# unionai-oss/unionml

Hardware: AMD Instinct MI355X
Metric: train_samples_per_sec (higher is better)
Workload: dtype bf16; 1 GPU; model=digits_mlp_64x32x10, global_batch=2048, parallelism=dp1, engine=fused+hipgraph64

## Files before the change

### unionml_amd/ops/hip/tabular_common.h

```cpp
#pragma once

#include <hip/hip_runtime.h>
#include <hip/hip_bf16.h>

#include "tabular_launch.h"

typedef __attribute__((ext_vector_type(8))) short bf16x8;
typedef __attribute__((ext_vector_type(4))) float f32x4;
typedef unsigned short u16;

constexpr int HEAD_XENT = 0;
constexpr int HEAD_REG = 1;

template <int HEAD> struct head_target { typedef int type; };
template <> struct head_target<HEAD_REG> { typedef float type; };
template <int HEAD> using head_target_t = typename head_target<HEAD>::type;

__device__ __forceinline__ float bf2f(u16 v) {
  union { float f; unsigned u; } c;
  c.u = ((unsigned)v) << 16;
  return c.f;
}

__device__ __forceinline__ u16 f2bf(float f) {
  union { float f; unsigned u; } c;
  c.f = f;
  unsigned lsb = (c.u >> 16) & 1u;
  c.u += 0x7fffu + lsb;
  return (u16)(c.u >> 16);
}

__device__ __forceinline__ float fast_rcp(float x) {
  return __builtin_amdgcn_rcpf(x);
}

template <int CTRL>
__device__ __forceinline__ float dpp_row_f32(float x) {
  return __int_as_float(__builtin_amdgcn_update_dpp(
      0, __float_as_int(x), CTRL, 0xF, 0xF, true));
}

__device__ __forceinline__ float row_sum16(float x) {
  x += dpp_row_f32<0xB1>(x);
  x += dpp_row_f32<0x4E>(x);
  x += dpp_row_f32<0x141>(x);
  x += dpp_row_f32<0x140>(x);
  return x;
}

template <int D>
__device__ __forceinline__ void group_pair(float x, float& a, float& b) {
  static_assert(D == 16 || D == 32, "row-of-16 or half-wave exchange");
  const int xi = __float_as_int(x);
  if constexpr (D == 16) {
    const auto r = __builtin_amdgcn_permlane16_swap(xi, xi, false, false);
    a = __int_as_float(r[0]);
    b = __int_as_float(r[1]);
  } else {
    const auto r = __builtin_amdgcn_permlane32_swap(xi, xi, false, false);
    a = __int_as_float(r[0]);
    b = __int_as_float(r[1]);
  }
}

template <int D>
__device__ __forceinline__ float group_sum(float x) {
  float a, b;
  group_pair<D>(x, a, b);
  return a + b;
}

template <int D>
__device__ __forceinline__ float group_max(float x) {
  float a, b;
  group_pair<D>(x, a, b);
  return fmaxf(a, b);
}


constexpr int tr_read_elem(int lane, int ks, int tile, int half, int stride) {
  const int lg = lane >> 4, lr = lane & 15;
  return (ks * 32 + lg * 8 + half * 4 + (lr >> 2)) * stride + tile * 16 + (lr & 3) * 4;
}

constexpr bool tr_read_map_ok(int stride, int KS, int TILES) {
  if (stride < TILES * 16) return false;
  for (int ks = 0; ks < KS; ++ks)
    for (int tile = 0; tile < TILES; ++tile)
      for (int half = 0; half < 2; ++half)
        for (int lane = 0; lane < 64; ++lane) {
          if ((tr_read_elem(lane, ks, tile, half, stride) * 2) % 8 != 0) return false;
          const int group = lane & ~15, i = lane & 15;
          for (int q = 0; q < 4; ++q) {
            const int got = tr_read_elem(group + 4 * q + (i >> 2), ks, tile, half, stride) + (i & 3);
            const int want_row = ks * 32 + (lane >> 4) * 8 + half * 4 + q;
            const int want_col = tile * 16 + i;
            if (got / stride != want_row || got % stride != want_col) return false;
          }
        }
  return true;
}

template <int STRIDE, int KS, int TILES>
__device__ __forceinline__ bf16x8 tr_read_k8(const u16 (*T)[STRIDE], int ks, int tile,
                                             int lane) {
  static_assert(tr_read_map_ok(STRIDE, KS, TILES), "transposed-read address map");
  typedef __attribute__((ext_vector_type(4))) short s16x4;
  typedef __attribute__((address_space(3))) s16x4 lds_s16x4;
  const u16* base = &T[0][0];
  const s16x4 lo = __builtin_amdgcn_ds_read_tr16_b64_v4i16(
      (lds_s16x4*)(base + tr_read_elem(lane, ks, tile, 0, STRIDE)));
  const s16x4 hi = __builtin_amdgcn_ds_read_tr16_b64_v4i16(
      (lds_s16x4*)(base + tr_read_elem(lane, ks, tile, 1, STRIDE)));
  return __builtin_shufflevector(lo, hi, 0, 1, 2, 3, 4, 5, 6, 7);
}


typedef __attribute__((address_space(1))) float xwg_f32;
typedef __attribute__((address_space(1))) unsigned xwg_u32;

__device__ __forceinline__ void xwg_store(float* p, float x) {
  __hip_atomic_store((xwg_f32*)p, x, __ATOMIC_RELAXED, __HIP_MEMORY_SCOPE_AGENT);
}
__device__ __forceinline__ void xwg_store(unsigned* p, unsigned x) {
  __hip_atomic_store((xwg_u32*)p, x, __ATOMIC_RELAXED, __HIP_MEMORY_SCOPE_AGENT);
}
__device__ __forceinline__ float xwg_load(const float* p) {
  return __hip_atomic_load((const xwg_f32*)p, __ATOMIC_RELAXED, __HIP_MEMORY_SCOPE_AGENT);
}
__device__ __forceinline__ unsigned xwg_load(const unsigned* p) {
  return __hip_atomic_load((const xwg_u32*)p, __ATOMIC_RELAXED, __HIP_MEMORY_SCOPE_AGENT);
}

__device__ __forceinline__ void xwg_store4(float* base, int n, int i, f32x4 x) {
  typedef __attribute__((ext_vector_type(4))) unsigned u32x4;
  const __amdgpu_buffer_rsrc_t rsrc =
      __builtin_amdgcn_make_buffer_rsrc(base, 0, n * 4, 0x00020000);
  __builtin_amdgcn_raw_buffer_store_b128(__builtin_bit_cast(u32x4, x), rsrc, i * 4, 0, 16);
}


__device__ __forceinline__ float adam_corr(float beta_pow_t) {
  return fast_rcp(1.f - beta_pow_t);
}

__device__ __forceinline__ void adam_bias_corr(float beta1, float beta2, float t,
                                               float& corr1, float& corr2) {
  corr1 = adam_corr(__powf(beta1, t));
  corr2 = adam_corr(__powf(beta2, t));
}

__device__ __forceinline__ void adam_update(float& p, float& m, float& v, float g,
                                            float lr, float beta1, float beta2,
                                            float eps, float corr1, float corr2) {
  const float omb1 = 1.f - beta1, omb2 = 1.f - beta2;
  float bm, bv, gs;
  {
    #pragma clang fp contract(off)
    bm = beta1 * m;
    bv = beta2 * v;
    gs = omb2 * g;
  }
  const float mi = __builtin_fmaf(omb1, g, bm);
  const float vi = __builtin_fmaf(g, gs, bv);
  m = mi;
  v = vi;
  p = p - lr * (mi * corr1) * fast_rcp(sqrtf(vi * corr2) + eps);
}


__device__ __forceinline__ void wimg_write(u16* __restrict__ wimg, int i, u16 wb) {
  static_assert(DIGITS_HID == 32 && DIGITS_CPAD == 16, "shifts below");
  if (i < DIGITS_OFF_B1) {
    const int in = i >> 5;
    const int h = i & 31;
    wimg[DIGITS_WIMG_W1T + h * DIGITS_XS + in] = wb;
  } else if (i >= DIGITS_OFF_W2 && i < DIGITS_OFF_B2) {
    const int j = i - DIGITS_OFF_W2;
    const int h = j >> 4;
    const int c = j & 15;
    wimg[DIGITS_WIMG_W2S + h * DIGITS_WS + c] = wb;
    wimg[DIGITS_WIMG_W2T + c * DIGITS_WS + h] = wb;
  }
}

__device__ __forceinline__ int wimg_w2s_off(int hid, int inp) { return hid * inp; }
__device__ __forceinline__ int wimg_w2t_off(int hid, int inp) {
  return hid * inp + hid * 32;
}

__device__ __forceinline__ void wimg_write_gen(u16* __restrict__ wimg, int inp,
                                               int hid, int cpad, int i, u16 wb) {
  const int off_b1 = inp * hid;
  const int off_w2 = off_b1 + hid;
  const int off_b2 = off_w2 + hid * cpad;
  if (i < off_b1) {
    wimg[(i % hid) * inp + (i / hid)] = wb;
  } else if (i >= off_w2 && i < off_b2) {
    const int j = i - off_w2;
    const int h = j / cpad, c = j % cpad;
    wimg[wimg_w2s_off(hid, inp) + h * 32 + c] = wb;
    wimg[wimg_w2t_off(hid, inp) + c * hid + h] = wb;
  }
}


template <int NCT>
__device__ __forceinline__ void head_logits(float (&logit)[NCT][4],
                                            const f32x4 (&acc)[NCT],
                                            const float* b2, int cls, int lg) {
  #pragma unroll
  for (int ct = 0; ct < NCT; ++ct) {
    #pragma unroll
    for (int r = 0; r < 4; ++r) {
      const int c = ct * 16 + lg * 4 + r;
      logit[ct][r] = (c < cls) ? acc[ct][r] + b2[c] : -1e30f;
    }
  }
}

__device__ __forceinline__ void head_logits_padded(float (&logit)[1][4],
                                                   const f32x4 (&acc)[1],
                                                   f32x4 b2v, int cls, int lg) {
  #pragma unroll
  for (int r = 0; r < 4; ++r) {
    const int c = lg * 4 + r;
    logit[0][r] = (c < cls) ? acc[0][r] + b2v[r] : -1e30f;
  }
}

template <int NCT>
__device__ __forceinline__ float head_row_max(const float (&logit)[NCT][4]) {
  float mx = -1e30f;
  #pragma unroll
  for (int ct = 0; ct < NCT; ++ct) {
    #pragma unroll
    for (int r = 0; r < 4; ++r) mx = fmaxf(mx, logit[ct][r]);
  }
  mx = group_max<16>(mx);
  mx = group_max<32>(mx);
  return mx;
}

template <int NCT>
__device__ __forceinline__ float head_exp_sum(float (&e)[NCT][4],
                                              const float (&logit)[NCT][4],
                                              float mx, int cls, int lg) {
  float s = 0.f;
  #pragma unroll
  for (int ct = 0; ct < NCT; ++ct) {
    #pragma unroll
    for (int r = 0; r < 4; ++r) {
      const int c = ct * 16 + lg * 4 + r;
      e[ct][r] = (c < cls) ? __expf(logit[ct][r] - mx) : 0.f;
      s += e[ct][r];
    }
  }
  s = group_sum<16>(s);
  s = group_sum<32>(s);
  return s;
}

template <int NCT>
__device__ __forceinline__ void head_argmax(const float (&logit)[NCT][4], int cls,
                                            int lg, float& best, int& bcol) {
  best = -1e30f;
  bcol = cls;
  #pragma unroll
  for (int ct = 0; ct < NCT; ++ct) {
    #pragma unroll
    for (int r = 0; r < 4; ++r) {
      if (logit[ct][r] > best) { best = logit[ct][r]; bcol = ct * 16 + lg * 4 + r; }
    }
  }
  #pragma unroll
  for (int d = 16; d < 64; d <<= 1) {
    const float ov = __shfl_xor(best, d, 64);
    const int oc = __shfl_xor(bcol, d, 64);
    if (ov > best || (ov == best && oc < bcol)) { best = ov; bcol = oc; }
  }
}
```

### unionml_amd/ops/hip/tabular_kernels.hip

```cpp

#include <hip/hip_runtime.h>

#include "tabular_common.h"

constexpr int IN = DIGITS_IN, HID = DIGITS_HID, CLS = DIGITS_CLS;
constexpr int CPAD = DIGITS_CPAD;
#define ROWS 128
#define WAVES 8
#define BLOCK (WAVES * 64)

constexpr int XS = DIGITS_XS;
#define HS 40
#define DHS 36
constexpr int WS = DIGITS_WS;


extern "C" __global__ void __launch_bounds__(256)
standardize_fit_fast_kernel(const float* __restrict__ X, long long N, int D,
                            double* __restrict__ scratch ) {
  const int tid = threadIdx.x;
  const int col = tid % D;
  const int rg = tid / D;
  const int rpi = 256 / D;
  double s = 0.0, s2 = 0.0;
  for (long long r = (long long)blockIdx.x * rpi + rg; r < N;
       r += (long long)gridDim.x * rpi) {
    const double v = (double)X[r * D + col];
    s += v;
    s2 += v * v;
  }
  __shared__ double ls[256], ls2[256];
  ls[tid] = s;
  ls2[tid] = s2;
  __syncthreads();
  for (int off = 128; off >= D; off >>= 1) {
    if (tid < off && tid + off < 256) {
      ls[tid] += ls[tid + off];
      ls2[tid] += ls2[tid + off];
    }
    __syncthreads();
  }
  if (tid < D) {
    atomicAdd(&scratch[col], ls[tid]);
    atomicAdd(&scratch[D + col], ls2[tid]);
  }
}

extern "C" __global__ void __launch_bounds__(256)
standardize_fit_finalize_kernel(const double* __restrict__ scratch, long long N,
                                int D, float* __restrict__ mean,
                                float* __restrict__ invstd, float eps) {
  const int col = blockIdx.x * blockDim.x + threadIdx.x;
  if (col >= D) return;
  const double m = scratch[col] / (double)N;
  const double var = scratch[D + col] / (double)N - m * m;
  mean[col] = (float)m;
  invstd[col] = (float)(1.0 / sqrt(var > 0.0 ? var + (double)eps : (double)eps));
}

extern "C" __global__ void __launch_bounds__(256)
standardize_fit_kernel(const float* __restrict__ X, long long N, int D,
                       float* __restrict__ mean, float* __restrict__ invstd,
                       float eps) {
  const int col = blockIdx.x;
  if (col >= D) return;
  double s = 0.0, s2 = 0.0;
  for (long long r = threadIdx.x; r < N; r += blockDim.x) {
    const double v = (double)X[r * D + col];
    s += v;
    s2 += v * v;
  }
  __shared__ double ls[256], ls2[256];
  ls[threadIdx.x] = s;
  ls2[threadIdx.x] = s2;
  __syncthreads();
  for (int off = 128; off > 0; off >>= 1) {
    if (threadIdx.x < off) {
      ls[threadIdx.x] += ls[threadIdx.x + off];
      ls2[threadIdx.x] += ls2[threadIdx.x + off];
    }
    __syncthreads();
  }
  if (threadIdx.x == 0) {
    const double m = ls[0] / (double)N;
    const double var = ls2[0] / (double)N - m * m;
    mean[col] = (float)m;
    invstd[col] = (float)(1.0 / sqrt(var > 0.0 ? var + (double)eps : (double)eps));
  }
}

extern "C" __global__ void __launch_bounds__(256)
standardize_apply_kernel(const float* __restrict__ X, long long n_elems, int D,
                         int Dout,
                         const float* __restrict__ mean,
                         const float* __restrict__ invstd,
                         u16* __restrict__ out) {
  for (long long i = (long long)blockIdx.x * blockDim.x + threadIdx.x; i < n_elems;
       i += (long long)gridDim.x * blockDim.x) {
    const int col = (int)(i % D);
    out[(i / D) * Dout + col] = f2bf((X[i] - mean[col]) * invstd[col]);
  }
}

constexpr int OFF_W1 = DIGITS_OFF_W1, OFF_B1 = DIGITS_OFF_B1;
constexpr int OFF_W2 = DIGITS_OFF_W2, OFF_B2 = DIGITS_OFF_B2;
constexpr int NPARAM = DIGITS_NPARAM, OFF_LOSS = NPARAM;
constexpr int SLAB = DIGITS_SLAB;


#define ALIGN16(x) (((x) + 15) & ~15)
#define C_XS   0
#define C_HS   ALIGN16(C_XS  + ROWS * XS * 2)
#define C_DLS  ALIGN16(C_HS  + ROWS * HS * 2)
#define C_DHS  ALIGN16(C_DLS + ROWS * HS * 2)
#define C_W1T  ALIGN16(C_DHS + ROWS * DHS * 2)
#define C_W2S  ALIGN16(C_W1T + HID * XS * 2)
#define C_W2T  ALIGN16(C_W2S + HID * WS * 2)
#define C_DB1  ALIGN16(C_W2T + CPAD * WS * 2)
#define C_DB2  ALIGN16(C_DB1 + HID * 4)
#define C_LOSS ALIGN16(C_DB2 + CPAD * 4)
#define C_B1S  ALIGN16(C_LOSS + 16)
#define C_B2S  ALIGN16(C_B1S + HID * 4)
#define NWAVE  (BLOCK / 64)
#define PART   (HID + CPAD + 1)
#define C_PART ALIGN16(C_B2S + CPAD * 4)
#define C_IMG_TOTAL ALIGN16(C_PART + NWAVE * PART * 4)
#define C_MASTER C_IMG_TOTAL
#define C_M    ALIGN16(C_MASTER + NPARAM * 4)
#define C_V    ALIGN16(C_M + NPARAM * 4)
#define C_STEPS_TOTAL ALIGN16(C_V + NPARAM * 4)

struct Lds {
  u16 (*Xs)[XS];
  u16 (*Hs)[HS];
  u16 (*DLs)[HS];
  u16 (*DHs)[DHS];
  u16 (*W1T)[XS];
  u16 (*W2s)[WS];
  u16 (*W2T)[WS];
  float* db1;
  float* db2;
  float* loss;
  float* b1s;
  float* b2s;
  float* part;
};

__device__ __forceinline__ Lds carve(char* smem) {
  Lds L;
  L.Xs = (u16(*)[XS])(smem + C_XS);
  L.Hs = (u16(*)[HS])(smem + C_HS);
  L.DLs = (u16(*)[HS])(smem + C_DLS);
  L.DHs = (u16(*)[DHS])(smem + C_DHS);
  L.W1T = (u16(*)[XS])(smem + C_W1T);
  L.W2s = (u16(*)[WS])(smem + C_W2S);
  L.W2T = (u16(*)[WS])(smem + C_W2T);
  L.db1 = (float*)(smem + C_DB1);
  L.db2 = (float*)(smem + C_DB2);
  L.loss = (float*)(smem + C_LOSS);
  L.b1s = (float*)(smem + C_B1S);
  L.b2s = (float*)(smem + C_B2S);
  L.part = (float*)(smem + C_PART);
  return L;
}

constexpr int WIMG_VECS = DIGITS_WIMG_N / 8;
constexpr int WIMG_TAIL = WIMG_VECS - BLOCK;
static_assert(WIMG_TAIL > 0 && WIMG_TAIL <= BLOCK, "two vectors per thread at most");

struct WimgRegs {
  bf16x8 v0, v1;
};

__device__ __forceinline__ void issue_weight_images_packed(
    WimgRegs& R, const u16* __restrict__ wimg) {
  const bf16x8* src = (const bf16x8*)wimg;
  const int tid = threadIdx.x;
  R.v0 = src[tid];
  R.v1 = src[tid < WIMG_TAIL ? BLOCK + tid : tid];
}

__device__ __forceinline__ void store_weight_images_packed(const WimgRegs& R,
                                                           const Lds& L) {
  bf16x8* dst = (bf16x8*)&L.W1T[0][0];
  const int tid = threadIdx.x;
  dst[tid] = R.v0;
  if (tid < WIMG_TAIL) dst[BLOCK + tid] = R.v1;
}

__device__ __forceinline__ float issue_biases(const float* __restrict__ b1,
                                              const float* __restrict__ b2) {
  const int tid = threadIdx.x;
  const float* p = tid < HID ? b1 + tid : tid < HID + CPAD ? b2 + (tid - HID) : b1;
  return *p;
}

template <typename T>
__device__ __forceinline__ T uniform_load(const T* p) {
  static_assert(sizeof(T) == 4, "one dword");
  typedef __attribute__((address_space(1))) const T gT;
  return __hip_atomic_load((gT*)p, __ATOMIC_RELAXED, __HIP_MEMORY_SCOPE_WAVEFRONT);
}

__device__ __forceinline__ void store_biases(float b, const Lds& L) {
  const int tid = threadIdx.x;
  if (tid < HID) L.b1s[tid] = b;
  else if (tid < HID + CPAD) L.b2s[tid - HID] = b;
}

__device__ __forceinline__ void load_weight_images(const Lds& L,
                                                   const u16* __restrict__ W1bf,
                                                   const u16* __restrict__ W2bf) {
  const int tid = threadIdx.x;
  for (int i = tid; i < HID * IN; i += BLOCK) {
    const int h = i / IN, k = i % IN;
    L.W1T[h][k] = W1bf[k * HID + h];
  }
  for (int i = tid; i < HID * 32; i += BLOCK) {
    const int h = i / 32, c = i % 32;
    L.W2s[h][c] = (c < CPAD) ? W2bf[h * CPAD + c] : (u16)0;
  }
  for (int i = tid; i < CPAD * HID; i += BLOCK) {
    const int c = i / HID, h = i % HID;
    L.W2T[c][h] = W2bf[h * CPAD + c];
  }
}

constexpr int X_VECS = ROWS * (IN / 8) / BLOCK;
static_assert(X_VECS * BLOCK == ROWS * (IN / 8), "whole vectors per thread");

struct XChunkRegs {
  bf16x8 v[X_VECS];
  bool vvalid[X_VECS];
  int label;
  bool valid;
};

__device__ __forceinline__ void issue_label(XChunkRegs& R,
                                            const int* __restrict__ y,
                                            long long row0, long long Nvalid) {
  const int tid = threadIdx.x;
  const long long row = row0 + (tid >> 6) * 16 + (tid & 15);
  R.valid = row < Nvalid;
  R.label = y[R.valid ? row : Nvalid - 1];
}

__device__ __forceinline__ void issue_x_chunk(XChunkRegs& R,
                                              const u16* __restrict__ Xbf,
                                              const int* __restrict__ y,
                                              long long row0, long long Nvalid) {
  const int tid = threadIdx.x;
  #pragma unroll
  for (int u = 0; u < X_VECS; ++u) {
    const int i = tid + u * BLOCK;
    const long long row = row0 + i / (IN / 8);
    const int c = (i % (IN / 8)) * 8;
    R.vvalid[u] = row < Nvalid;
    R.v[u] = *(const bf16x8*)&Xbf[(R.vvalid[u] ? row : Nvalid - 1) * IN + c];
  }
  issue_label(R, y, row0, Nvalid);
}

__device__ __forceinline__ int chunk_label(const XChunkRegs& R) {
  return R.valid ? R.label : -1;
}

__device__ __forceinline__ void store_x_chunk(const XChunkRegs& R, const Lds& L) {
  const int tid = threadIdx.x;
  #pragma unroll
  for (int u = 0; u < X_VECS; ++u) {
    const int i = tid + u * BLOCK;
    const int r = i / (IN / 8);
    const int c = (i % (IN / 8)) * 8;
    const bf16x8 v = R.vvalid[u] ? R.v[u] : (bf16x8){0, 0, 0, 0, 0, 0, 0, 0};
    *(bf16x8*)&L.Xs[r][c] = v;
  }
}

__device__ __forceinline__ void zero_dl_pad(const Lds& L) {
  static_assert(2 * ROWS <= BLOCK && CPAD == 16 && (HS * 2) % 16 == 0, "one b128 store per thread");
  const int t = threadIdx.x;
  if (t < 2 * ROWS) *(bf16x8*)&L.DLs[t >> 1][CPAD + (t & 1) * 8] = (bf16x8){0, 0, 0, 0, 0, 0, 0, 0};
}

typedef __attribute__((ext_vector_type(2))) unsigned u32x2;
__device__ __forceinline__ void store_bf16x4(u16* p, const u16 (&x)[4]) {
  *(u32x2*)p = (u32x2){(unsigned)x[0] | ((unsigned)x[1] << 16),
                       (unsigned)x[2] | ((unsigned)x[3] << 16)};
}

struct ChunkAcc {
  f32x4 dW1;
  f32x4 dW2;
};

constexpr int BIAS_SUM_T0 = (NWAVE - 1) * 64;

template <bool SINGLE>
__device__ __forceinline__ void chunk_fwd_bwd(
    const Lds& L, const float* b1, const float* b2,
    const int label, const bool valid, float invBtot, ChunkAcc& acc_io,
    float& bias_sum) {
  const int tid = threadIdx.x;
  const int wave = tid >> 6;
  const int l = tid & 63;
  const int lg = l >> 4, lr = l & 15;
  const int wrow = wave * 16;

  bf16x8 w1f[HID / 16][IN / 32], xf[IN / 32];
  f32x4 b1v[HID / 16];
  #pragma unroll
  for (int mt = 0; mt < HID / 16; ++mt) b1v[mt] = *(const f32x4*)&b1[mt * 16 + lg * 4];
  const f32x4 b2v = *(const f32x4*)&b2[lg * 4];
  __builtin_amdgcn_sched_barrier(0);
  #pragma unroll
  for (int ks = 0; ks < IN / 32; ++ks) {
    xf[ks] = *(const bf16x8*)&L.Xs[wrow + lr][ks * 32 + lg * 8];
    #pragma unroll
    for (int mt = 0; mt < HID / 16; ++mt) {
      w1f[mt][ks] = *(const bf16x8*)&L.W1T[mt * 16 + lr][ks * 32 + lg * 8];
    }
  }
  __builtin_amdgcn_sched_barrier(0);

  u16 hbits[HID / 16][4];
  f32x4 hacc[HID / 16];
  #pragma unroll
  for (int mt = 0; mt < HID / 16; ++mt) {
    hacc[mt] = (f32x4){0.f, 0.f, 0.f, 0.f};
    #pragma unroll
    for (int ks = 0; ks < IN / 32; ++ks) {
      hacc[mt] = __builtin_amdgcn_mfma_f32_16x16x32_bf16(w1f[mt][ks], xf[ks], hacc[mt], 0, 0, 0);
    }
  }
  #pragma unroll
  for (int mt = 0; mt < HID / 16; ++mt) {
    #pragma unroll
    for (int r = 0; r < 4; ++r) {
      float hv = hacc[mt][r] + b1v[mt][r];
      hv = hv > 0.f ? hv : 0.f;
      const u16 hb = f2bf(hv);
      hbits[mt][r] = hb;
    }
    store_bf16x4(&L.Hs[wrow + lr][mt * 16 + lg * 4], hbits[mt]);
  }
  asm volatile("s_waitcnt lgkmcnt(0)" ::: "memory");

  {
    f32x4 acc[1] = {{0.f, 0.f, 0.f, 0.f}};
    const bf16x8 a = *(const bf16x8*)&L.W2T[lr][lg * 8];
    const bf16x8 b = *(const bf16x8*)&L.Hs[wrow + lr][lg * 8];
    acc[0] = __builtin_amdgcn_mfma_f32_16x16x32_bf16(a, b, acc[0], 0, 0, 0);

    const int row = wrow + lr;

    float logit[1][4], e[1][4];
    head_logits_padded(logit, acc, b2v, CLS, lg);
    const float m = head_row_max<1>(logit);
    const float s = head_exp_sum<1>(e, logit, m, CLS, lg);
    const float rs = fast_rcp(s);
    const float logs = __logf(s);
    float db2_acc[4];
    float loss_acc = 0.f;
    u16 dlbits[4];
    #pragma unroll
    for (int r = 0; r < 4; ++r) {
      const int c = lg * 4 + r;
      const float dl = valid ? (e[0][r] * rs - (c == label ? 1.f : 0.f)) * invBtot : 0.f;
      const u16 dlb = f2bf(dl);
      dlbits[r] = dlb;
      db2_acc[r] = dl;
      if (valid && c == label) loss_acc = -(logit[0][r] - m - logs) * invBtot;
    }
    store_bf16x4(&L.DLs[row][lg * 4], dlbits);
    #pragma unroll
    for (int r = 0; r < 4; ++r) db2_acc[r] = row_sum16(db2_acc[r]);
    loss_acc = row_sum16(loss_acc);
    loss_acc = group_sum<16>(loss_acc);
    loss_acc = group_sum<32>(loss_acc);
    if (lr == 0) {
      #pragma unroll
      for (int r = 0; r < 4; ++r) L.part[wave * PART + HID + lg * 4 + r] = db2_acc[r];
      if (l == 0) L.part[wave * PART + HID + CPAD] = loss_acc;
    }
  }
  asm volatile("s_waitcnt lgkmcnt(0)" ::: "memory");

  {
    float db1_acc[HID / 16][4];
    #pragma unroll
    for (int mt = 0; mt < HID / 16; ++mt) {
      f32x4 acc = {0.f, 0.f, 0.f, 0.f};
      const bf16x8 a = *(const bf16x8*)&L.W2s[mt * 16 + lr][lg * 8];
      const bf16x8 b = *(const bf16x8*)&L.DLs[wrow + lr][lg * 8];
      acc = __builtin_amdgcn_mfma_f32_16x16x32_bf16(a, b, acc, 0, 0, 0);
      u16 dhbits[4];
      #pragma unroll
      for (int r = 0; r < 4; ++r) {
        const float hv = bf2f(hbits[mt][r]);
        const float dh = hv > 0.f ? acc[r] : 0.f;
        dhbits[r] = f2bf(dh);
        db1_acc[mt][r] = dh;
      }
      store_bf16x4(&L.DHs[wrow + lr][mt * 16 + lg * 4], dhbits);
    }
    #pragma unroll
    for (int mt = 0; mt < HID / 16; ++mt) {
      #pragma unroll
      for (int r = 0; r < 4; ++r) db1_acc[mt][r] = row_sum16(db1_acc[mt][r]);
    }
    if (lr == 0) {
      #pragma unroll
      for (int mt = 0; mt < HID / 16; ++mt) {
        #pragma unroll
        for (int r = 0; r < 4; ++r) {
          L.part[wave * PART + mt * 16 + lg * 4 + r] = db1_acc[mt][r];
        }
      }
    }
  }
  __syncthreads();

  bias_sum = 0.f;
  if (wave == NWAVE - 1 && l < PART) {
    float sum = 0.f;
    #pragma unroll
    for (int w = 0; w < NWAVE; ++w) sum += L.part[w * PART + l];
    if constexpr (SINGLE) {
      bias_sum = 0.f + sum;
    } else {
      if (l < HID) L.db1[l] += sum;
      else if (l < HID + CPAD) L.db2[l - HID] += sum;
      else L.loss[0] += sum;
    }
  }

  {
    const int ht = wave & 1, it = wave >> 1;
    bf16x8 a[ROWS / 32], b[ROWS / 32];
    #pragma unroll
    for (int ks = 0; ks < ROWS / 32; ++ks) {
      a[ks] = tr_read_k8<DHS, ROWS / 32, HID / 16>(L.DHs, ks, ht, l);
      b[ks] = tr_read_k8<XS, ROWS / 32, IN / 16>(L.Xs, ks, it, l);
    }
    __builtin_amdgcn_sched_barrier(0);
    f32x4 acc = acc_io.dW1;
    #pragma unroll
    for (int ks = 0; ks < ROWS / 32; ++ks) {
      acc = __builtin_amdgcn_mfma_f32_16x16x32_bf16(a[ks], b[ks], acc, 0, 0, 0);
    }
    acc_io.dW1 = acc;
  }
  if (wave < 2) {
    bf16x8 a[ROWS / 32], b[ROWS / 32];
    #pragma unroll
    for (int ks = 0; ks < ROWS / 32; ++ks) {
      a[ks] = tr_read_k8<HS, ROWS / 32, HID / 16>(L.Hs, ks, wave, l);
      b[ks] = tr_read_k8<HS, ROWS / 32, CPAD / 16>(L.DLs, ks, 0, l);
    }
    __builtin_amdgcn_sched_barrier(0);
    f32x4 acc = acc_io.dW2;
    #pragma unroll
    for (int ks = 0; ks < ROWS / 32; ++ks) {
      acc = __builtin_amdgcn_mfma_f32_16x16x32_bf16(a[ks], b[ks], acc, 0, 0, 0);
    }
    acc_io.dW2 = acc;
  }
  if constexpr (!SINGLE) __syncthreads();
}

__device__ __forceinline__ int bias_sum_index(int i) {
  return i < HID ? OFF_B1 + i : i < HID + CPAD ? OFF_B2 + (i - HID) : OFF_LOSS;
}


extern "C" __global__ void __launch_bounds__(BLOCK)
mlp_step_kernel(const u16* __restrict__ Xbf, const int* __restrict__ y, int B,
                const u16* __restrict__ W1bf, const u16* __restrict__ W2bf,
                const float* __restrict__ master,
                float* __restrict__ grads, float invBtot) {
  extern __shared__ __attribute__((aligned(16))) char smem[];
  const Lds L = carve(smem);

  const int tid = threadIdx.x;
  const int wave = tid >> 6;
  const int l = tid & 63;
  const int lg = l >> 4, lr = l & 15;
  const long long row0 = (long long)blockIdx.x * ROWS;

  XChunkRegs xr;
  issue_x_chunk(xr, Xbf, y, row0, B);
  const float bias = issue_biases(master + OFF_B1, master + OFF_B2);
  zero_dl_pad(L);
  load_weight_images(L, W1bf, W2bf);
  store_x_chunk(xr, L);
  store_biases(bias, L);
  __syncthreads();

  ChunkAcc acc;
  acc.dW1 = (f32x4){0.f, 0.f, 0.f, 0.f};
  acc.dW2 = (f32x4){0.f, 0.f, 0.f, 0.f};
  float bias_sum;
  chunk_fwd_bwd<true>(L, L.b1s, L.b2s, chunk_label(xr), xr.valid, invBtot, acc, bias_sum);

  {
    const int ht = wave & 1, it = wave >> 1;
    #pragma unroll
    for (int r = 0; r < 4; ++r) {
      const int h = ht * 16 + lg * 4 + r;
      const int in = it * 16 + lr;
      atomicAdd(&grads[OFF_W1 + in * HID + h], acc.dW1[r]);
    }
  }
  if (wave < 2) {
    #pragma unroll
    for (int r = 0; r < 4; ++r) {
      const int h = wave * 16 + lg * 4 + r;
      atomicAdd(&grads[OFF_W2 + h * CPAD + lr], acc.dW2[r]);
    }
  }
  if (tid >= BIAS_SUM_T0 && tid < BIAS_SUM_T0 + PART) {
    atomicAdd(&grads[bias_sum_index(tid - BIAS_SUM_T0)], bias_sum);
  }
}


extern "C" __global__ void __launch_bounds__(BLOCK)
mlp_step_fused_kernel(
                      const u16* __restrict__ Xbf, const int* __restrict__ y,
                      int B,
                      u16* __restrict__ wimg,
                      float* __restrict__ master,
                      unsigned* __restrict__ counter,
                      int* __restrict__ t_dev,
                      const u16* __restrict__ W1bf, const u16* __restrict__ W2bf,
                      u16* __restrict__ bfmirror,
                      float* __restrict__ m, float* __restrict__ v,
                      float* __restrict__ slabs,
                      float* __restrict__ loss_out,
                      float invBtot, float lr, float beta1, float beta2,
                      float eps,
                      float* __restrict__ grads_out) {
  asm volatile("" :: "s"(Xbf), "s"(y), "s"(B), "s"(wimg), "s"(master), "s"(counter),
               "s"(t_dev));

  extern __shared__ __attribute__((aligned(16))) char smem[];
  const Lds L = carve(smem);
  unsigned* lossu = (unsigned*)L.loss;

  const int tid = threadIdx.x;
  const int wave = tid >> 6;
  const int l = tid & 63;
  const int lg = l >> 4, lr_ = l & 15;
  const long long row0 = (long long)blockIdx.x * ROWS;

  XChunkRegs xr;
  WimgRegs wr;
#ifndef PROBE_SKIP_LOADS
  issue_x_chunk(xr, Xbf, y, row0, B);
  if (wimg) issue_weight_images_packed(wr, wimg);
#else
  issue_label(xr, y, row0, B);
#endif
  const float bias = issue_biases(master + OFF_B1, master + OFF_B2);
  const unsigned counter_pre = uniform_load(counter);
  const unsigned t_pre = (unsigned)uniform_load(t_dev);
  const int n_wg = gridDim.x;
  asm volatile("" :: "s"(W1bf), "s"(W2bf), "s"(bfmirror), "s"(m), "s"(v), "s"(slabs),
               "s"(loss_out), "s"(invBtot), "s"(lr), "s"(beta1), "s"(beta2), "s"(eps),
               "s"(grads_out), "s"(n_wg));

  zero_dl_pad(L);
#ifndef PROBE_SKIP_LOADS
  if (wimg) store_weight_images_packed(wr, L);
  else load_weight_images(L, W1bf, W2bf);
  store_x_chunk(xr, L);
#endif
  store_biases(bias, L);
  const unsigned epoch = counter_pre + 1u;
  asm volatile("" :: "v"(epoch), "v"(t_pre));
  __syncthreads();

  ChunkAcc acc;
  acc.dW1 = (f32x4){0.f, 0.f, 0.f, 0.f};
  acc.dW2 = (f32x4){0.f, 0.f, 0.f, 0.f};
  float bias_sum = 0.f;
#ifndef PROBE_SKIP_FWDBWD
  chunk_fwd_bwd<true>(L, L.b1s, L.b2s, chunk_label(xr), xr.valid, invBtot, acc, bias_sum);
#endif

  float* slab = slabs + (long long)blockIdx.x * SLAB;
  {
    static_assert(OFF_W1 % 4 == 0 && HID % 4 == 0 && SLAB % 4 == 0, "16-B dW1 stores");
    const int ht = wave & 1, it = wave >> 1;
    const int in = it * 16 + lr_;
    xwg_store4(slab, SLAB, OFF_W1 + in * HID + ht * 16 + lg * 4, acc.dW1);
  }
  if (wave < 2) {
    #pragma unroll
    for (int r = 0; r < 4; ++r) {
      const int h = wave * 16 + lg * 4 + r;
      xwg_store(&slab[OFF_W2 + h * CPAD + lr_], acc.dW2[r]);
    }
  }
  if (tid >= BIAS_SUM_T0 && tid < BIAS_SUM_T0 + PART) {
    xwg_store(&slab[bias_sum_index(tid - BIAS_SUM_T0)], bias_sum);
  }

  float* pre = (float*)L.Xs;
  const int span_pre = (NPARAM + 1 + n_wg - 1) / n_wg;
  const int lo_pre = blockIdx.x * span_pre;
  const bool use_pre =
      (grads_out == nullptr) && (3 * span_pre * 4 <= ROWS * XS * 2);
#ifndef PROBE_SKIP_HANDSHAKE
  asm volatile("s_waitcnt vmcnt(0)" ::: "memory");
  __syncthreads();
  if (tid == 0) xwg_store((unsigned*)(slab + NPARAM + 1), epoch);

  if (use_pre) {
    const int hi_pre = min(lo_pre + span_pre, NPARAM);
    for (int i = lo_pre + tid; i < hi_pre; i += BLOCK) {
      const int j = i - lo_pre;
      pre[j] = master[i];
      pre[span_pre + j] = m[i];
      pre[2 * span_pre + j] = v[i];
    }
  }

  if (wave == 0) {
    unsigned spins = 0;
    bool ok = true;
    for (int w = l; w < n_wg; w += 64) {
      for (;;) {
        const unsigned tag = xwg_load(
            (const unsigned*)(slabs + (long long)w * SLAB + NPARAM + 1));
        if (tag == epoch) break;
        __builtin_amdgcn_s_sleep(2);
        if (++spins > 100000000u) { ok = false; break; }
      }
      if (!ok) break;
    }
    const unsigned long long bad = __ballot(!ok);
    __builtin_amdgcn_fence(__ATOMIC_ACQUIRE, "wavefront");
    if (l == 0) lossu[1] = bad ? 1u : 0u;
  }
  __syncthreads();
  if (lossu[1] != 0u) {
    if (tid == 0 && blockIdx.x == 0) *loss_out = __builtin_nanf("");
    return;
  }
#endif

#ifdef PROBE_SKIP_REDUCE
  if (tid == 0 && blockIdx.x == 0) {
    *counter = epoch;
    if (!grads_out) *t_dev = (int)(t_pre + 1u);
  }
  return;
#endif
  const float t_new = (float)(t_pre + 1u);
  float corr1, corr2;
  adam_bias_corr(beta1, beta2, t_new, corr1, corr2);
  const int span = (NPARAM + 1 + n_wg - 1) / n_wg;
  const int lo = blockIdx.x * span;
  const int hi = min(lo + span, NPARAM + 1);
  for (int i = lo + tid; i < hi; i += BLOCK) {
    float gc[8] = {0.f, 0.f, 0.f, 0.f, 0.f, 0.f, 0.f, 0.f};
    int w = 0;
    for (; w + 16 <= n_wg; w += 16) {
      float a[16];
      #pragma unroll
      for (int k = 0; k < 16; ++k) a[k] = xwg_load(&slabs[(long long)(w + k) * SLAB + i]);
      #pragma unroll
      for (int k = 0; k < 16; ++k) gc[k & 7] += a[k];
    }
    for (; w + 8 <= n_wg; w += 8) {
      float a[8];
      #pragma unroll
      for (int k = 0; k < 8; ++k) a[k] = xwg_load(&slabs[(long long)(w + k) * SLAB + i]);
      #pragma unroll
      for (int k = 0; k < 8; ++k) gc[k] += a[k];
    }
    if (w < n_wg) {
      float a[7];
      #pragma unroll
      for (int k = 0; k < 7; ++k) {
        a[k] = xwg_load(&slabs[(long long)min(w + k, n_wg - 1) * SLAB + i]);
      }
      #pragma unroll
      for (int k = 0; k < 7; ++k) {
        if (w + k < n_wg) gc[0] += a[k];
      }
    }
    const float g0 = gc[0], g1 = gc[1], g2 = gc[2], g3 = gc[3];
    const float g4 = gc[4], g5 = gc[5], g6 = gc[6], g7 = gc[7];
    const float g = ((g0 + g1) + (g2 + g3)) + ((g4 + g5) + (g6 + g7));
    if (grads_out) {
      grads_out[i] = g;
      continue;
    }
    if (i == NPARAM) {
      *loss_out = g;
      continue;
    }
    const int j = i - lo;
    float p = use_pre ? pre[j] : master[i];
    float mi = use_pre ? pre[span_pre + j] : m[i];
    float vi = use_pre ? pre[2 * span_pre + j] : v[i];
    adam_update(p, mi, vi, g, lr, beta1, beta2, eps, corr1, corr2);
    m[i] = mi;
    v[i] = vi;
    master[i] = p;
    const u16 wb = f2bf(p);
    bfmirror[i] = wb;
    if (wimg) wimg_write(wimg, i, wb);
  }
  if (tid == 0 && blockIdx.x == 0) {
    *counter = epoch;
    if (!grads_out) *t_dev = (int)t_new;
  }
}


extern "C" __global__ void __launch_bounds__(256)
adam_step_kernel(float* __restrict__ master, u16* __restrict__ bfmirror,
                 const float* __restrict__ grads, float* __restrict__ m,
                 float* __restrict__ v, int* __restrict__ t_dev,
                 float lr, float beta1, float beta2, float eps,
                 u16* __restrict__ wimg) {
  __shared__ float corr1, corr2;
  if (threadIdx.x == 0) {
    const int t = ++(*t_dev);
    adam_bias_corr(beta1, beta2, (float)t, corr1, corr2);
  }
  __syncthreads();
  for (int base = (int)threadIdx.x; base < NPARAM; base += 256 * 4) {
    float g[4], mi_[4], vi_[4], p_[4];
    int idx[4], n = 0;
    #pragma unroll
    for (int u = 0; u < 4; ++u) {
      const int i = base + u * 256;
      if (i < NPARAM) {
        idx[n] = i;
        g[n] = grads[i];
        mi_[n] = m[i];
        vi_[n] = v[i];
        p_[n] = master[i];
        ++n;
      }
    }
    #pragma unroll
    for (int u = 0; u < 4; ++u) {
      if (u < n) {
        float p = p_[u], mi = mi_[u], vi = vi_[u];
        adam_update(p, mi, vi, g[u], lr, beta1, beta2, eps, corr1, corr2);
        const int i = idx[u];
        m[i] = mi;
        v[i] = vi;
        master[i] = p;
        const u16 wb = f2bf(p);
        bfmirror[i] = wb;
        if (wimg) wimg_write(wimg, i, wb);
      }
    }
  }
}


extern "C" __global__ void __launch_bounds__(BLOCK, 1)
mlp_train_steps_kernel(const u16* __restrict__ Xbf,
                       const int* __restrict__ y,
                       long long N, int B, int n_steps,
                       float* __restrict__ master,
                       u16* __restrict__ bfmirror,
                       float* __restrict__ m,
                       float* __restrict__ v,
                       int* __restrict__ t_dev,
                       float* __restrict__ loss_out,
                       float lr, float beta1, float beta2, float eps) {
  extern __shared__ __attribute__((aligned(16))) char smem[];
  const Lds L = carve(smem);
  float* master_s = (float*)(smem + C_MASTER);
  float* m_s = (float*)(smem + C_M);
  float* v_s = (float*)(smem + C_V);

  const int tid = threadIdx.x;
  const int wave = tid >> 6;
  const int l = tid & 63;
  const int lg = l >> 4, ln = l & 15;

  for (int i = tid; i < NPARAM; i += BLOCK) {
    master_s[i] = master[i];
    m_s[i] = m[i];
    v_s[i] = v[i];
  }
  __syncthreads();
  for (int i = tid; i < HID * IN; i += BLOCK) {
    const int h = i / IN, k = i % IN;
    L.W1T[h][k] = f2bf(master_s[OFF_W1 + k * HID + h]);
  }
  for (int i = tid; i < HID * 32; i += BLOCK) {
    const int h = i / 32, c = i % 32;
    L.W2s[h][c] = (c < CPAD) ? f2bf(master_s[OFF_W2 + h * CPAD + c]) : (u16)0;
  }
  for (int i = tid; i < CPAD * HID; i += BLOCK) {
    const int c = i / HID, h = i % HID;
    L.W2T[c][h] = f2bf(master_s[OFF_W2 + h * CPAD + c]);
  }
  zero_dl_pad(L);
  const int t0 = *t_dev;
  float b1t = __powf(beta1, (float)t0), b2t = __powf(beta2, (float)t0);
  __syncthreads();

  const int batches = (int)(N / B);
  const int chunks = B / ROWS;
  const float invB = fast_rcp((float)B);

  for (int s = 0; s < n_steps; ++s) {
    const long long base = (long long)(s % batches) * B;

    if (tid < HID) L.db1[tid] = 0.f;
    if (tid < CPAD) L.db2[tid] = 0.f;
    if (tid == 0) L.loss[0] = 0.f;

    ChunkAcc acc;
    acc.dW1 = (f32x4){0.f, 0.f, 0.f, 0.f};
    acc.dW2 = (f32x4){0.f, 0.f, 0.f, 0.f};

    for (int ch = 0; ch < chunks; ++ch) {
      const long long row0 = base + (long long)ch * ROWS;
      XChunkRegs xr;
      issue_x_chunk(xr, Xbf, y, row0, N);
      store_x_chunk(xr, L);
      __syncthreads();
      float unused;
      chunk_fwd_bwd<false>(L, master_s + OFF_B1, master_s + OFF_B2, chunk_label(xr),
                           xr.valid, invB, acc, unused);
    }

    b1t *= beta1;
    b2t *= beta2;
    const float corr1 = adam_corr(b1t);
    const float corr2 = adam_corr(b2t);

    auto adam_at = [&](int i, float g) {
      adam_update(master_s[i], m_s[i], v_s[i], g, lr, beta1, beta2, eps, corr1, corr2);
    };

    {
      const int ht = wave & 1, it = wave >> 1;
      #pragma unroll
      for (int r = 0; r < 4; ++r) {
        const int h = ht * 16 + lg * 4 + r;
        const int in = it * 16 + ln;
        const int idx = OFF_W1 + in * HID + h;
        adam_at(idx, acc.dW1[r]);
        L.W1T[h][in] = f2bf(master_s[idx]);
      }
    }
    if (wave < 2) {
      #pragma unroll
      for (int r = 0; r < 4; ++r) {
        const int h = wave * 16 + lg * 4 + r;
        const int idx = OFF_W2 + h * CPAD + ln;
        adam_at(idx, acc.dW2[r]);
        const u16 wb = f2bf(master_s[idx]);
        L.W2s[h][ln] = wb;
        L.W2T[ln][h] = wb;
      }
    }
    if (wave == 2) {
      if (l < HID) {
        adam_at(OFF_B1 + l, L.db1[l]);
      } else if (l < HID + CPAD) {
        adam_at(OFF_B2 + (l - HID), L.db2[l - HID]);
      }
    }
    __syncthreads();
  }

  if (tid == 0) {
    *t_dev = t0 + n_steps;
    *loss_out = L.loss[0];
  }
  for (int i = tid; i < NPARAM; i += BLOCK) {
    master[i] = master_s[i];
    m[i] = m_s[i];
    v[i] = v_s[i];
    bfmirror[i] = f2bf(master_s[i]);
  }
}


extern "C" __global__ void __launch_bounds__(BLOCK)
mlp_predict_kernel(const float* __restrict__ X, int B,
                   const float* __restrict__ mean,
                   const float* __restrict__ invstd,
                   const u16* __restrict__ W1bf, const u16* __restrict__ W2bf,
                   const float* __restrict__ master,
                   int* __restrict__ preds,
                   float* __restrict__ probs ) {
  extern __shared__ __attribute__((aligned(16))) char smem[];
  const Lds L = carve(smem);

  const int tid = threadIdx.x;
  const int wave = tid >> 6;
  const int l = tid & 63;
  const int lg = l >> 4, lr = l & 15;
  const long long row0 = (long long)blockIdx.x * ROWS;
  const int wrow = wave * 16;

  for (int i = tid; i < ROWS * IN; i += BLOCK) {
    const int r = i / IN, c = i % IN;
    const float v =
        (row0 + r < B) ? (X[(row0 + r) * IN + c] - mean[c]) * invstd[c] : 0.f;
    L.Xs[r][c] = f2bf(v);
  }
  load_weight_images(L, W1bf, W2bf);
  __syncthreads();

  const float* b1 = master + OFF_B1;
  const float* b2 = master + OFF_B2;

  #pragma unroll
  for (int mt = 0; mt < HID / 16; ++mt) {
    f32x4 acc = {0.f, 0.f, 0.f, 0.f};
    #pragma unroll
    for (int ks = 0; ks < IN / 32; ++ks) {
      const bf16x8 a = *(const bf16x8*)&L.W1T[mt * 16 + lr][ks * 32 + lg * 8];
      const bf16x8 b = *(const bf16x8*)&L.Xs[wrow + lr][ks * 32 + lg * 8];
      acc = __builtin_amdgcn_mfma_f32_16x16x32_bf16(a, b, acc, 0, 0, 0);
    }
    #pragma unroll
    for (int r = 0; r < 4; ++r) {
      const int h = mt * 16 + lg * 4 + r;
      float hv = acc[r] + b1[h];
      L.Hs[wrow + lr][h] = f2bf(hv > 0.f ? hv : 0.f);
    }
  }
  __syncthreads();

  {
    f32x4 acc[1] = {{0.f, 0.f, 0.f, 0.f}};
    const bf16x8 a = *(const bf16x8*)&L.W2T[lr][lg * 8];
    const bf16x8 b = *(const bf16x8*)&L.Hs[wrow + lr][lg * 8];
    acc[0] = __builtin_amdgcn_mfma_f32_16x16x32_bf16(a, b, acc[0], 0, 0, 0);

    const int row = wrow + lr;
    float best;
    int bcol;
    float logit[1][4];
    head_logits<1>(logit, acc, b2, CLS, lg);
    head_argmax<1>(logit, CLS, lg, best, bcol);
    if (lg == 0 && row0 + row < B) preds[row0 + row] = bcol;
    if (probs != nullptr) {
      float e[1][4];
      const float rs = fast_rcp(head_exp_sum<1>(e, logit, best, CLS, lg));
      #pragma unroll
      for (int r = 0; r < 4; ++r) {
        const int c = lg * 4 + r;
        if (c < CLS && row0 + row < B) {
          probs[(row0 + row) * CLS + c] = e[0][r] * rs;
        }
      }
    }
  }
}


extern "C" __global__ void __launch_bounds__(64)
reduce_selftest_kernel(const float* __restrict__ x, int n,
                       float* __restrict__ out) {
  const int row = blockIdx.x;
  const int l = threadIdx.x;
  if (row >= n) return;
  const float v = x[(long long)row * 64 + l];
  const float dpp = row_sum16(v);
  float bfly = v;
  bfly += __shfl_xor(bfly, 1, 64);
  bfly += __shfl_xor(bfly, 2, 64);
  bfly += __shfl_xor(bfly, 4, 64);
  bfly += __shfl_xor(bfly, 8, 64);
  out[((long long)row * 64 + l) * 2 + 0] = dpp;
  out[((long long)row * 64 + l) * 2 + 1] = bfly;
}


extern "C" {

void launch_standardize_fit(const float* X, long long N, int D, float* mean,
                            float* invstd, float eps, double* scratch,
                            hipStream_t stream) {
  if (scratch != nullptr && D <= 256 && 256 % D == 0) {
    const int rpi = 256 / D;
    long long blocks_ll = (N * (long long)D * 4) / 65536;
    int blocks = (int)(blocks_ll < 1 ? 1 : (blocks_ll > 1024 ? 1024 : blocks_ll));
    {
      const int max_useful = (int)((N + rpi - 1) / rpi);
      if (blocks > max_useful) blocks = max_useful;
    }
    hipLaunchKernelGGL(standardize_fit_fast_kernel, dim3(blocks), dim3(256), 0,
                       stream, X, N, D, scratch);
    hipLaunchKernelGGL(standardize_fit_finalize_kernel,
                       dim3((D + 255) / 256), dim3(256), 0, stream, scratch, N,
                       D, mean, invstd, eps);
    return;
  }
  hipLaunchKernelGGL(standardize_fit_kernel, dim3(D), dim3(256), 0, stream,
                     X, N, D, mean, invstd, eps);
}

void launch_standardize_apply(const float* X, long long N, int D, int Dout,
                              const float* mean, const float* invstd,
                              unsigned short* out, hipStream_t stream) {
  const long long n = N * D;
  int blocks = (int)((n + 255) / 256);
  if (blocks > 2048) blocks = 2048;
  hipLaunchKernelGGL(standardize_apply_kernel, dim3(blocks), dim3(256), 0, stream,
                     X, n, D, Dout, mean, invstd, out);
}

int launch_mlp_step(const unsigned short* Xbf, const int* y, int B,
                    const unsigned short* W1bf, const unsigned short* W2bf,
                    const float* master, float* grads, float invBtot,
                    hipStream_t stream) {
  if (B < 1) return -3;
  if (ensure_dynamic_lds<mlp_step_kernel>(C_IMG_TOTAL) != 0) return -2;
  const int blocks = (B + ROWS - 1) / ROWS;
  hipLaunchKernelGGL(mlp_step_kernel, dim3(blocks), dim3(BLOCK), C_IMG_TOTAL,
                     stream, Xbf, y, B, W1bf, W2bf, master, grads, invBtot);
  return 0;
}

int launch_mlp_step_fused(const unsigned short* Xbf, const int* y, int B,
                          const unsigned short* W1bf, const unsigned short* W2bf,
                          float* master, unsigned short* bfmirror, float* m,
                          float* v, int* t_dev, float* slabs, unsigned* counter,
                          float* loss_out, float invBtot, float lr, float beta1,
                          float beta2, float eps, int max_slabs, float* grads_out,
                          unsigned short* wimg, hipStream_t stream) {
  if (B < 1) return -3;
  const int blocks = (B + ROWS - 1) / ROWS;
  if (blocks > max_slabs) return -1;
  if (ensure_dynamic_lds<mlp_step_fused_kernel>(C_IMG_TOTAL) != 0) return -2;
  hipLaunchKernelGGL(mlp_step_fused_kernel, dim3(blocks), dim3(BLOCK), C_IMG_TOTAL,
                     stream, Xbf, y, B, wimg, master, counter, t_dev, W1bf, W2bf,
                     bfmirror, m, v, slabs, loss_out, invBtot, lr, beta1, beta2, eps,
                     grads_out);
  return 0;
}

int launch_mlp_train_steps(const unsigned short* Xbf, const int* y, long long N,
                           int B, int n_steps, float* master,
                           unsigned short* bfmirror, float* m, float* v,
                           int* t_dev, float* loss_out, float lr, float beta1,
                           float beta2, float eps, hipStream_t stream) {
  if (B < 1 || N < 1 || n_steps < 0) return -3;
  if (B % ROWS != 0 || N % B != 0) return -1;
  if (ensure_dynamic_lds<mlp_train_steps_kernel>(C_STEPS_TOTAL) != 0) return -2;
  hipLaunchKernelGGL(mlp_train_steps_kernel, dim3(1), dim3(BLOCK), C_STEPS_TOTAL,
                     stream, Xbf, y, N, B, n_steps, master, bfmirror, m, v,
                     t_dev, loss_out, lr, beta1, beta2, eps);
  return 0;
}

int launch_mlp_predict(const float* X, int B, const float* mean,
                       const float* invstd, const unsigned short* W1bf,
                       const unsigned short* W2bf, const float* master,
                       int* preds, float* probs, hipStream_t stream) {
  if (B < 1) return -3;
  if (ensure_dynamic_lds<mlp_predict_kernel>(C_IMG_TOTAL) != 0) return -2;
  const int blocks = (B + ROWS - 1) / ROWS;
  hipLaunchKernelGGL(mlp_predict_kernel, dim3(blocks), dim3(BLOCK), C_IMG_TOTAL,
                     stream, X, B, mean, invstd, W1bf, W2bf, master, preds, probs);
  return 0;
}

void launch_adam_step(float* master, unsigned short* bfmirror, const float* grads,
                      float* m, float* v, int* t_dev, float lr, float beta1,
                      float beta2, float eps, unsigned short* wimg,
                      hipStream_t stream) {
  hipLaunchKernelGGL(adam_step_kernel, dim3(1), dim3(256), 0, stream,
                     master, bfmirror, grads, m, v, t_dev, lr, beta1, beta2, eps,
                     wimg);
}

void launch_reduce_selftest(const float* x, int n, float* out,
                            hipStream_t stream) {
  if (n <= 0) return;
  hipLaunchKernelGGL(reduce_selftest_kernel, dim3(n), dim3(64), 0, stream, x, n,
                     out);
}

}
```

Measured before the change: 280.5 million samples/s.

## Overlap Adam prefetch and bias-correction with cross-workgroup handshake polling

In the fused step kernel, wave 0 now only polls the cross-workgroup handshake while waves 1..7 prefetch master/m/v into LDS and compute the Adam bias-correction factors (wave 1 for beta1, wave 2 for beta2), which are passed through LDS. The reduction/update loop is restriped over the non-polling waves only. The standalone adam_step_kernel also issues its first batch of loads before the bias-correction sync and software-pipelines later batches. The aim is to hide the power/reciprocal and global-load latency behind the spin wait, at the cost of one fewer wave doing the reduce/update work.

```diff
diff --git a/unionml_amd/ops/hip/tabular_common.h b/unionml_amd/ops/hip/tabular_common.h
--- a/unionml_amd/ops/hip/tabular_common.h
+++ b/unionml_amd/ops/hip/tabular_common.h
@@ -144,10 +144,14 @@
   return fast_rcp(1.f - beta_pow_t);
 }
 
+__device__ __forceinline__ float adam_bias_corr_one(float beta, float t) {
+  return adam_corr(__powf(beta, t));
+}
+
 __device__ __forceinline__ void adam_bias_corr(float beta1, float beta2, float t,
                                                float& corr1, float& corr2) {
-  corr1 = adam_corr(__powf(beta1, t));
-  corr2 = adam_corr(__powf(beta2, t));
+  corr1 = adam_bias_corr_one(beta1, t);
+  corr2 = adam_bias_corr_one(beta2, t);
 }
 
 __device__ __forceinline__ void adam_update(float& p, float& m, float& v, float g,
diff --git a/unionml_amd/ops/hip/tabular_kernels.hip b/unionml_amd/ops/hip/tabular_kernels.hip
--- a/unionml_amd/ops/hip/tabular_kernels.hip
+++ b/unionml_amd/ops/hip/tabular_kernels.hip
@@ -525,6 +525,10 @@
 }
 
 
+constexpr int STRIPE_T0 = 64;
+constexpr int STRIPE_STEP = BLOCK - STRIPE_T0;
+__device__ __forceinline__ int stripe_first(int lo, int tid) { return lo + (tid - STRIPE_T0); }
+
 extern "C" __global__ void __launch_bounds__(BLOCK)
 mlp_step_fused_kernel(
                       const u16* __restrict__ Xbf, const int* __restrict__ y,
@@ -612,22 +616,47 @@
   const int lo_pre = blockIdx.x * span_pre;
   const bool use_pre =
       (grads_out == nullptr) && (3 * span_pre * 4 <= ROWS * XS * 2);
+  const float t_new = (float)(t_pre + 1u);
+  float corr1 = 0.f, corr2 = 0.f;
 #ifndef PROBE_SKIP_HANDSHAKE
   asm volatile("s_waitcnt vmcnt(0)" ::: "memory");
   __syncthreads();
   if (tid == 0) xwg_store((unsigned*)(slab + NPARAM + 1), epoch);
 
-  if (use_pre) {
+  if (wave != 0) {
     const int hi_pre = min(lo_pre + span_pre, NPARAM);
-    for (int i = lo_pre + tid; i < hi_pre; i += BLOCK) {
+    int i = stripe_first(lo_pre, tid);
+    const bool first = use_pre && i < hi_pre;
+    float p0 = 0.f, m0 = 0.f, v0 = 0.f;
+    if (first) {
+      p0 = master[i];
+      m0 = m[i];
+      v0 = v[i];
+    }
+    if (!grads_out && wave <= 2) {
+#ifdef PROBE_CONST_CORR
+      const float c = wave == 1 ? 10.f : 1000.f;
+#else
+      const float c = adam_bias_corr_one(wave == 1 ? beta1 : beta2, t_new);
+#endif
+      asm volatile("" :: "v"(c));
+      if (l == 0) L.loss[1 + wave] = c;
+    }
+    if (first) {
       const int j = i - lo_pre;
-      pre[j] = master[i];
-      pre[span_pre + j] = m[i];
-      pre[2 * span_pre + j] = v[i];
-    }
-  }
-
-  if (wave == 0) {
+      pre[j] = p0;
+      pre[span_pre + j] = m0;
+      pre[2 * span_pre + j] = v0;
+    }
+    if (use_pre) {
+      for (i += STRIPE_STEP; i < hi_pre; i += STRIPE_STEP) {
+        const int j = i - lo_pre;
+        pre[j] = master[i];
+        pre[span_pre + j] = m[i];
+        pre[2 * span_pre + j] = v[i];
+      }
+    }
+  } else {
     unsigned spins = 0;
     bool ok = true;
     for (int w = l; w < n_wg; w += 64) {
@@ -640,6 +669,16 @@
       }
       if (!ok) break;
     }
+#ifdef PROBE_COUNT_POLLS
+    {
+      unsigned rounds = spins + 1u;
+      #pragma unroll
+      for (int o = 32; o > 0; o >>= 1) rounds = max(rounds, (unsigned)__shfl_xor((int)rounds, o));
+      if (l == 0 && blockIdx.x == 0) {
+        atomicAdd((unsigned*)(slabs + NPARAM + 2) + (min(rounds, 14u) - 1u), 1u);
+      }
+    }
+#endif
     const unsigned long long bad = __ballot(!ok);
     __builtin_amdgcn_fence(__ATOMIC_ACQUIRE, "wavefront");
     if (l == 0) lossu[1] = bad ? 1u : 0u;
@@ -658,13 +697,15 @@
   }
   return;
 #endif
-  const float t_new = (float)(t_pre + 1u);
-  float corr1, corr2;
-  adam_bias_corr(beta1, beta2, t_new, corr1, corr2);
+#ifdef PROBE_SKIP_HANDSHAKE
+  if (!grads_out) adam_bias_corr(beta1, beta2, t_new, corr1, corr2);
+#else
+  if (!grads_out) corr1 = L.loss[2], corr2 = L.loss[3];
+#endif
   const int span = (NPARAM + 1 + n_wg - 1) / n_wg;
   const int lo = blockIdx.x * span;
   const int hi = min(lo + span, NPARAM + 1);
-  for (int i = lo + tid; i < hi; i += BLOCK) {
+  for (int i = stripe_first(lo, tid); wave != 0 && i < hi; i += STRIPE_STEP) {
     float gc[8] = {0.f, 0.f, 0.f, 0.f, 0.f, 0.f, 0.f, 0.f};
     int w = 0;
     for (; w + 16 <= n_wg; w += 16) {
@@ -729,32 +770,36 @@
                  float lr, float beta1, float beta2, float eps,
                  u16* __restrict__ wimg) {
   __shared__ float corr1, corr2;
-  if (threadIdx.x == 0) {
-    const int t = ++(*t_dev);
-    adam_bias_corr(beta1, beta2, (float)t, corr1, corr2);
-  }
-  __syncthreads();
-  for (int base = (int)threadIdx.x; base < NPARAM; base += 256 * 4) {
-    float g[4], mi_[4], vi_[4], p_[4];
-    int idx[4], n = 0;
-    #pragma unroll
-    for (int u = 0; u < 4; ++u) {
+  constexpr int U = 4, STEP = 256 * U;
+  float g[U], mi_[U], vi_[U], p_[U];
+  auto load_batch = [&](int base) {
+    #pragma unroll
+    for (int u = 0; u < U; ++u) {
       const int i = base + u * 256;
       if (i < NPARAM) {
-        idx[n] = i;
-        g[n] = grads[i];
-        mi_[n] = m[i];
-        vi_[n] = v[i];
-        p_[n] = master[i];
-        ++n;
-      }
-    }
-    #pragma unroll
-    for (int u = 0; u < 4; ++u) {
-      if (u < n) {
+        g[u] = grads[i];
+        mi_[u] = m[i];
+        vi_[u] = v[i];
+        p_[u] = master[i];
+      }
+    }
+  };
+  int t = 0;
+  if (threadIdx.x == 0) t = *t_dev + 1;
+  int base = (int)threadIdx.x;
+  load_batch(base);
+  if (threadIdx.x == 0) {
+    *t_dev = t;
+    adam_bias_corr(beta1, beta2, (float)t, corr1, corr2);
+  }
+  __syncthreads();
+  for (;;) {
+    #pragma unroll
+    for (int u = 0; u < U; ++u) {
+      const int i = base + u * 256;
+      if (i < NPARAM) {
         float p = p_[u], mi = mi_[u], vi = vi_[u];
         adam_update(p, mi, vi, g[u], lr, beta1, beta2, eps, corr1, corr2);
-        const int i = idx[u];
         m[i] = mi;
         v[i] = vi;
         master[i] = p;
@@ -763,6 +808,9 @@
         if (wimg) wimg_write(wimg, i, wb);
       }
     }
+    base += STEP;
+    if (base >= NPARAM) break;
+    load_batch(base);
   }
 }
 
```

Measured after the change: 302.6 million samples/s (median of 6 runs). 1.08x the previous value.
